# yoyololicon/spectrogram-inversion

Hardware: AMD Instinct MI355X
Metric: Griffin-Lim iterations*frames/sec at n_fft=2048 hop=512 (higher is better)
Workload: dtype f32; 1 GPU; C2: griffin_lim B64/GPU n_fft=2048 hop=512 T=1024 it=100 alpha=0.3 hann center reflect tol=0 eva_iter=10; global_batch=64, parallelism=batch-sharded x1, RCCL gather, step=phase_init + ISTFT + iterations + gather, kernel=k_fused4_td

## Files before the change

### spectrogram_inversion_amd/csrc/fast_core.h

```cpp
#pragma once
#include <algorithm>
#include <cstdlib>
#include <vector>

#include "common.h"
#include "kernels_generic.h"


namespace specinv {
namespace fast {

constexpr int kMinWaves = 2;
constexpr int kFused4Waves = 8;
constexpr int kR8Waves = 3;
constexpr double kTdsFloor = 9.3132257461547852e-10;

using v2f = float __attribute__((ext_vector_type(2)));
using v4f = float __attribute__((ext_vector_type(4)));

enum { MODE_GLA = 0, MODE_ADMM = 1 };

__device__ __forceinline__ v2f cmul_k(v2f a, v2f b) { return v2f{a.x * b.x - a.y * b.y, a.x * b.y + a.y * b.x}; }
__device__ __forceinline__ v2f cmulc_k(v2f a, v2f b) { return v2f{a.x * b.x + a.y * b.y, a.y * b.x - a.x * b.y}; }
__device__ __forceinline__ v2f cmul(v2f a, v2f b) {
// ... 531 lines not shown
  if (G::C == 4 && PK) {
#pragma unroll
    for (int g = 0; g < R; g += 4) {
      z[g] = tr[k.tr_q + (0 * R + g) * (R + 1)];
      z[g + 2] = tr[k.tr_q + (1 * R + g) * (R + 1)];
      z[g + 1] = tr[k.tr_q + (2 * R + g) * (R + 1)];
      z[g + 3] = tr[k.tr_q + (3 * R + g) * (R + 1)];
    }
#pragma unroll
    for (int g = 0; g < R; g += 4) {
      z[g + 2] = cmulc_p<PK>(z[g + 2], k.postq[0]);
      z[g + 1] = cmulc_p<PK>(z[g + 1], k.postq[1]);
      z[g + 3] = cmulc_p<PK>(z[g + 3], k.postq[2]);
    }
#pragma unroll
    for (int g = 0; g < R; g += 4) xlane_dft4_out<true>(z[g], z[g + 1], z[g + 2], z[g + 3]);
    cmul_all<R, PK, true, 1>(z, tw);
    Dft<R, true, PKC>::run(z);
    return;
  }
#pragma unroll
  for (int i = 0; i < R; ++i) z[i] = tr[k.tr_a + i * (R + 1)];
  cmul_all<R, PK, true, 0>(z, SameW{k.post});
  if (G::C == 2) {
#pragma unroll
    for (int g = 0; g < R; g += 2) xlane_dft2(z[g], z[g + 1]);
  } else if (G::C == 4) {
#pragma unroll
    for (int g = 0; g < R; g += 4) xlane_dft4<true>(z[g], z[g + 1], z[g + 2], z[g + 3]);
  } else if (G::C == 16) {
    const float s3 = (k.lane & 8) ? -1.0f : 1.0f, s2 = (k.lane & 4) ? -1.0f : 1.0f;
#pragma unroll
    for (int i = 0; i < R; ++i) {
      z[i] = cmulc_p<PK>(xlane_bf2(z[i], 4, s2), k.stage[1]);
      z[i] = cmulc_p<PK>(xlane_bf2(z[i], 8, s3), k.stage[0]);
    }
#pragma unroll
    for (int g = 0; g < R; g += 4) xlane_dft4<true>(z[g], z[g + 1], z[g + 2], z[g + 3]);
  } else {
    const bool upper = k.v & 1;
    const float sg = upper ? -1.0f : 1.0f;
#pragma unroll
    for (int i = 0; i < R; ++i) {
      const v2f p = shfl_xor2(z[i], R);
      z[i] = v2f{fmaf(z[i].x, sg, p.x), fmaf(z[i].y, sg, p.y)};
      z[i] = cmulc_p<PK>(z[i], k.stage[0]);
    }
#pragma unroll
    for (int g = 0; g < R; g += 4) xlane_dft4<true>(z[g], z[g + 1], z[g + 2], z[g + 3]);
  }
  cmul_all<R, PK, true, 1>(z, tw);
  Dft<R, true, PKC>::run(z);
}

__device__ __forceinline__ v2f w64(int j) {
  constexpr float tab[16][2] = {{1.000000000e+00f, -0.000000000e+00f}, {9.951847267e-01f, -9.801714033e-02f}, {9.807852804e-01f, -1.950903220e-01f}, {9.569403357e-01f, -2.902846773e-01f}, {9.238795325e-01f, -3.826834324e-01f}, {8.819212643e-01f, -4.713967368e-01f}, {8.314696123e-01f, -5.555702330e-01f}, {7.730104534e-01f, -6.343932842e-01f}, {7.071067812e-01f, -7.071067812e-01f}, {6.343932842e-01f, -7.730104534e-01f}, {5.555702330e-01f, -8.314696123e-01f}, {4.713967368e-01f, -8.819212643e-01f}, {3.826834324e-01f, -9.238795325e-01f}, {2.902846773e-01f, -9.569403357e-01f}, {1.950903220e-01f, -9.807852804e-01f}, {9.801714033e-02f, -9.951847267e-01f}};
  return v2f{tab[j][0], tab[j][1]};
}

struct FastArgs {
  const float* x_in;
  float* x_out;
  const float* xtail_in;
  float* xtail_out;
  const v4f* P_in;
  v4f* P_out;
  const v2f* Pmid_in;
  v2f* Pmid_out;
  v4f* X_out;
  v4f* U_out;
  v2f* Xmid_out;
  v2f* Umid_out;
  const v4f* m_pairs;
  const float* m_mid;
  const float* window;
  const float* env;
  double* partials;
  int T, nchunks, n_waves, pad_mode;
  long long L;
  const float* x2_in;
  float* x2_out;
  float tds;
  int skew;
  float coef;
  float inv1p;
  float fwd_scale;
  float inv_scale;
  v4f* P2_out;
  v2f* Pmid2_out;
  const v4f* m2_pairs;
  const float* m2_mid;
};

__device__ __forceinline__ float fast_abs(v2f s) { return __builtin_amdgcn_sqrtf(fmaf(s.x, s.x, s.y * s.y)); }
__device__ __forceinline__ float fast_rcp(float v) { return __builtin_amdgcn_rcpf(v); }
constexpr float kRefFloor = 1e-32f;
__device__ __forceinline__ float ref_norm2(v2f s, float floor_ = kRefFloor) { return fmaf(s.y, s.y, fmaf(s.x, s.x, floor_)); }
__device__ __forceinline__ v2f ref_rcp_abs2(v2f t, float guard = 1e-16f) {
  const v2f y = v2f{__builtin_amdgcn_rsqf(t.x), __builtin_amdgcn_rsqf(t.y)};
  v2f h = t * y;
  const v2f e = __builtin_elementwise_fma(-h, y, v2f{1.0f, 1.0f});
  return __builtin_elementwise_fma(y * 0.5f, e, y);
}
__device__ __forceinline__ float ref_rcp_abs(float t, float guard = 1e-16f) {
  const float y = __builtin_amdgcn_rsqf(t);
  float h = t * y;
  return fmaf(y * 0.5f, fmaf(-h, y, 1.0f), y);
}
__device__ __forceinline__ float env_rcp(float e) {
  const float r = __builtin_amdgcn_rcpf(e);
  return fmaf(fmaf(-e, r, 1.0f), r, r);
}
__device__ __forceinline__ v2f env_rcp(v2f e) { return v2f{env_rcp(e.x), env_rcp(e.y)}; }
__device__ __forceinline__ v2f env_apply_r(v2f v, v2f e, v2f r) {
  const v2f q = v * r;
  return __builtin_elementwise_fma(__builtin_elementwise_fma(-q, e, v), r, q);
}
__device__ __forceinline__ v2f env_apply(v2f v, v2f e) { return v2f{__fdiv_rn(v.x, e.x), __fdiv_rn(v.y, e.y)}; }
__device__ __forceinline__ float env_apply(float v, float e) { return __fdiv_rn(v, e); }

template <int MODE, bool EVAL>
__device__ __forceinline__ v2f update_bin(v2f r, v2f& p, v2f& u, v2f& xs, float m, const FastArgs& a, bool live, double& sd,
                                          double& so) {
  if (EVAL) {
    const float o = fast_abs(r);
    if (live) {
      const double d = (double)o - (double)m;
      sd += d * d;
      so += (double)o * (double)o;
    }
  }
  if (MODE == MODE_GLA) {
    const v2f s = v2f{fmaf(-a.coef, p.x, r.x), fmaf(-a.coef, p.y, r.y)};
    p = s;
    return ((s * m) * ref_rcp_abs(ref_norm2(s))) * a.inv_scale;
  } else {
    const v2f y = p;
    const v2f z = v2f{fmaf(a.coef, y.x, r.x) * a.inv1p, fmaf(a.coef, y.y, r.y) * a.inv1p};
    const v2f un = y - z;
    v2f xn = z - un;
    {
#pragma clang fp contract(off)
      xn = (xn * m) * ref_rcp_abs(ref_norm2(xn));
    }
    xs = xn;
    u = un;
    p = xn + un;
    return p * a.inv_scale;
  }
}

__device__ __forceinline__ long long pad_index(long long n, long long L, int pad_mode) {
  if (n >= 0 && n < L) return n;
  switch (pad_mode) {
    case SPECINV_PAD_REFLECT:
      return n < 0 ? -n : 2 * (L - 1) - n;
    case SPECINV_PAD_REPLICATE:
      return n < 0 ? 0 : L - 1;
    case SPECINV_PAD_CIRCULAR:
      return n < 0 ? n + L : n - L;
    default:
      return -1;
  }
}

__device__ __host__ __forceinline__ int chunk_begin(int c, int T, int nchunks, int skew = 0) {
// ... 228 lines not shown
```

### spectrogram_inversion_amd/csrc/fast_state.h

```cpp
#pragma once
#include <algorithm>
#include "dev_buf.h"
#include "fast_core.h"
#include "kernels_layout.h"

namespace specinv {

template <typename T>
struct FastState {
  bool supported = false;
  bool semi = false;
  bool hopk = false;
  bool xform_ok = false;
  bool two = false;
  bool keep_state = false;
  bool plain_state = false;
  int n_partials = 0;
  int nchunks = 0, skew = 0, OV = 0;
  int max_partials() const { return 0; }
  T* state_rows() const { return nullptr; }
  const T* state_tails() const { return nullptr; }
  int setup(const specinv_stft_cfg&, const std::vector<T>&, int64_t, int) { return SPECINV_OK; }
  void geometry(int out[4]) const { out[0] = out[1] = out[2] = out[3] = 0; }
  template <typename P>
  int launch_xform(P&, bool, const T*, long long, void*, T*, T, int = -1) { return fail(SPECINV_EUNSUPPORTED, "no fused path"); }
  template <typename P>
  int launch_inverse_ola(P&, const void*, T*, long long, T, T**, bool* used) {
    *used = false;
    return SPECINV_OK;
  }
  template <typename P>
  int begin(P&, int, const void*, const void*, double*) { return fail(SPECINV_EUNSUPPORTED, "no fused path for this dtype"); }
  template <typename P>
  int iterate(P&, int, bool) { return fail(SPECINV_EUNSUPPORTED, "no fused path for this dtype"); }
  template <typename P>
  int get_wave(P&, T*) { return fail(SPECINV_EUNSUPPORTED, "no fused path for this dtype"); }
  template <typename P>
  int get_state_spec(P&, int, cplx<T>*) { return fail(SPECINV_EUNSUPPORTED, "no fused path for this dtype"); }
};

#define SPECINV_R_SWITCH(RV, ...)                      \
  switch (RV) {                                        \
    case 4: { constexpr int RR = 4; __VA_ARGS__; } break;   \
    case 8: { constexpr int RR = 8; __VA_ARGS__; } break;   \
    case 16: { constexpr int RR = 16; __VA_ARGS__; } break; \
    default: { constexpr int RR = 32; __VA_ARGS__; } break; \
  }

#define SPECINV_EARLY_EVAL(early, ev, K, ...)                                                                     \
  ((early) ? ((ev) ? (const void*)K<__VA_ARGS__, true, true> : (const void*)K<__VA_ARGS__, true, false>)          \
           : ((ev) ? (const void*)K<__VA_ARGS__, false, true> : (const void*)K<__VA_ARGS__, false, false>))

struct FastKnobs {
  bool disable_fast = false;
  bool disable_twosided = false;
  bool disable_fused = false;
  bool disable_hop = false;
  bool fused_template = false;
  bool eval_kernel = true;
  bool debug = false;
  bool has_small_frames = false;
  long long small_frames = 0;
  int fast_chunk = 0;
  int cu_budget = 0;
  bool has_k4_skew = false;
  int k4_s1 = 0, k4_s2 = 0;
  bool has_td_skew = false;
  int td_skew = 0;

  static FastKnobs read() {
    auto starts = [](const char* name, char c) {
      const char* e = getenv(name);
      return e != nullptr && e[0] == c;
    };
    FastKnobs k;
    k.disable_fast = starts("SPECINV_DISABLE_FAST", '1');
    k.disable_twosided = starts("SPECINV_DISABLE_TWOSIDED", '1');
    k.disable_fused = starts("SPECINV_DISABLE_FUSED", '1');
    k.disable_hop = starts("SPECINV_DISABLE_HOP", '1');
    k.fused_template = starts("SPECINV_FUSED_TEMPLATE", '1');
    k.eval_kernel = !starts("SPECINV_EVAL_KERNEL", '0');
    k.debug = getenv("SPECINV_DEBUG") != nullptr;
    if (const char* e = getenv("SPECINV_SMALL_FRAMES")) {
      k.has_small_frames = true;
      k.small_frames = atoll(e);
    }
    if (const char* e = getenv("SPECINV_FAST_CHUNK")) k.fast_chunk = atoi(e);
    if (const char* e = getenv("SPECINV_CU_BUDGET")) k.cu_budget = atoi(e);
    if (const char* e = getenv("SPECINV_K4_SKEW")) k.has_k4_skew = sscanf(e, "%d,%d", &k.k4_s1, &k.k4_s2) == 2;
    if (const char* e = getenv("SPECINV_TD_SKEW")) {
      k.has_td_skew = true;
      k.td_skew = atoi(e);
    }
    return k;
  }
  long long frames_from(long long measured) const { return has_small_frames ? small_frames : measured; }
};

inline double chunk_cost(int batch, int n_frames, int nch, long long slots) {
  const long long waves = (long long)batch * nch;
  const long long rounds = (waves + slots - 1) / slots;
  const int longest = (n_frames + nch - 1) / nch;
  return (double)rounds * (longest + 2.0) * (1.0 + 0.0015 * std::max(0, longest - 32));
}
struct ChunkPick {
  int nch = 0;
  double cost = 1e300;
};
inline ChunkPick pick_chunks(int batch, int n_frames, long long slots, int lo, int hi, int mult = 1, double tie = 1e-9) {
  ChunkPick best;
  for (int nch = lo; nch <= hi; ++nch) {
    if (nch % mult != 0) continue;
    const double cost = chunk_cost(batch, n_frames, nch, slots);
    if (cost < best.cost + tie) best = ChunkPick{nch, cost};
  }
  return best;
}

enum FastKernel {
  kKernelFused4 = 1,
  kKernelFused = 2,
  kKernelSemi = 3,
  kKernelHop = 4,
  kKernelFused4Td = 5,
  kKernelFusedTd = 6,
  kKernelHopTd = 7,
};

template <>
struct FastState<float> {
  using v2f = fast::v2f;
  using v4f = fast::v4f;
  bool supported = false;
  bool semi = false;
  bool hopk = false;
  int semi_grid = 0;
  int R = 0;
  int OV = 0;
  FastKnobs knobs;
  int chunk = 32, nchunks = 0, n_waves = 0, n_partials = 0;
  int skew = 0;
  int cur = 0;
  int mode = fast::MODE_GLA;
  DevBuf xb[2], xtail[2], Pb, Pmid, mpairs, mmid, scratch;
  bool two = false;
  DevBuf Pb2, Pmid2, mpairs2, mmid2;
  bool keep_state = false, xu_valid = false;
  DevBuf Xb, Xmid, Ub, Umid;
  bool plain_state = false;
  float* state_rows() const { return xb[cur].template as<float>(); }
  const float* state_tails() const { return (!semi && nchunks > 1) ? xtail[cur].template as<float>() : nullptr; }
  bool td = false;
  int td_t = 0;
  DevBuf zb[2];

  template <typename P>
  int want_xu(P& pl, fast::FastArgs& a, bool last) {
    if (mode != fast::MODE_ADMM) return SPECINV_OK;
    xu_valid = false;
    if (!keep_state || !last) return SPECINV_OK;
    SI_TRY(reserve_xu(pl));
    a.X_out = Xb.template as<v4f>();
    a.U_out = Ub.template as<v4f>();
    a.Xmid_out = Xmid.template as<v2f>();
// ... 19 lines not shown
    if (cfg.dtype != SPECINV_F32) return SPECINV_OK;
    knobs = FastKnobs::read();
    if (knobs.disable_fast) return SPECINV_OK;
    const bool size_ok = cfg.n_fft == 512 || cfg.n_fft == 1024 || cfg.n_fft == 2048 || cfg.n_fft == 4096;
    if (!size_ok) return SPECINV_OK;
    if (!cfg.onesided) {
      if (knobs.disable_twosided) return SPECINV_OK;
      if (pad >= length) return SPECINV_OK;
      two = true;
    } else {
      xform_ok = true;
      xform_R = cfg.n_fft / 128;
    }
    R = cfg.n_fft / 128;
    semi = false;
    OV = 0;
    for (int o : {2, 4, 8})
      if (cfg.hop_length * o == cfg.n_fft && R % o == 0) OV = o;
    if (two || knobs.disable_fused) OV = 0;
    const long long n_all = (long long)cfg.batch * cfg.n_frames;
    const bool small = n_all < knobs.frames_from(6144);
    if (!cfg.center || OV == 0 || cfg.n_frames < OV + 2 || pad >= length || small) {
      semi = true;
      hopk = false;
      OV = 0;
      chunk = cfg.n_frames;
      nchunks = 1;
      semi_grid = (int)std::min<long long>((n_all + 3) / 4, 256 * 8);
      n_waves = semi_grid * 4;
      supported = true;
      const bool want_hop = !knobs.disable_hop && R <= 16 && n_all >= knobs.frames_from(R >= 16 ? 12288 : 32768) && !small &&
                            cfg.hop_length >= 1 && cfg.hop_length <= cfg.n_fft && pad < length;
      if (want_hop) {
        const int floor_ch = std::max(8, (cfg.n_fft - 1) / cfg.hop_length + 1);
        const long long slots = R >= 16 ? 2048 : R == 8 ? 4096 : 6144;
        hopk = true;
        nchunks = pick_chunks(cfg.batch, cfg.n_frames, slots, 1, std::max(1, cfg.n_frames / floor_ch)).nch;
        if (knobs.fast_chunk >= 1) nchunks = std::max(1, cfg.n_frames / std::min(std::max(knobs.fast_chunk, floor_ch), cfg.n_frames));
        chunk = (cfg.n_frames + nchunks - 1) / nchunks;
        n_waves = cfg.batch * nchunks;
        if (knobs.debug) fprintf(stderr, "specinv: frame kernel with LDS overlap-add R=%d hop=%d chunks=%d of <=%d frames, %d waves\n", R, cfg.hop_length, nchunks, chunk, n_waves);
      }
      return SPECINV_OK;
    }
    const int floor_ch = OV == 8 ? 16 : 8;
    long long slots = 1024LL * (R >= 32 ? 1 : R <= 4 ? 3 : 2);
    if (R == 8) slots = 1024LL * fast::kR8Waves;
    if (knobs.cu_budget > 0 && knobs.cu_budget < 256) slots = slots * (256 - knobs.cu_budget) / 256;
    const int most = std::max(1, cfg.n_frames / floor_ch);
    ChunkPick best = pick_chunks(cfg.batch, cfg.n_frames, slots, 1, most);
    if (OV == 4 && (R == 16 || R == 8)) {
      const int mult = R == 16 ? 2 : 3;
      if (best.nch % mult != 0) {
        const ChunkPick pick = pick_chunks(cfg.batch, cfg.n_frames, slots, std::max(mult, best.nch - mult), std::min(best.nch + mult, most), mult, 0.0);
        if (pick.nch > 0 && pick.cost <= 1.04 * best.cost) best = pick;
      }
    }
    nchunks = best.nch;
    if (knobs.fast_chunk >= 4) nchunks = std::max(1, cfg.n_frames / std::min(std::max(knobs.fast_chunk, OV == 8 ? 13 : 4), cfg.n_frames));
    chunk = (cfg.n_frames + nchunks - 1) / nchunks;
    n_waves = cfg.batch * nchunks;
    if (knobs.debug) fprintf(stderr, "specinv: fused R=%d OV=%d chunks=%d of <=%d frames, %d waves (%lld slots)\n", R, OV, nchunks, chunk, n_waves, slots);
    supported = true;
    return SPECINV_OK;
  }

  template <typename P>
  fast::FastArgs base_args(P& pl) const {
    fast::FastArgs a{};
    a.m_pairs = mpairs.template as<v4f>();
    a.m_mid = mmid.template as<float>();
    if (two) {
      a.P2_out = Pb2.template as<v4f>();
      a.Pmid2_out = Pmid2.template as<v2f>();
      a.m2_pairs = mpairs2.template as<v4f>();
      a.m2_mid = mmid2.template as<float>();
    }
    a.window = pl.window.template as<float>();
    a.env = pl.env.template as<float>();
    a.partials = pl.partials_out();
    a.T = pl.Tn();
    a.nchunks = nchunks;
    a.skew = skew;
    a.n_waves = n_waves;
    a.pad_mode = pl.cfg.pad_mode;
    a.L = pl.length;
    a.coef = pl.coef;
    a.inv1p = 1.0f / (float)(1.0 + (double)pl.coef);
    a.fwd_scale = pl.fc.fwd_scale;
    a.inv_scale = pl.fc.inv_scale;
    return a;
  }

  template <typename P, typename A>
  static int launch_waves(P& pl, const void* fn, const A& args, int waves, int wgw, size_t lds) {
    SI_HIP(hipFuncSetAttribute(fn, hipFuncAttributeMaxDynamicSharedMemorySize, (int)lds));
    A copy = args;
    void* kargs[] = {&copy};
    SI_HIP(hipLaunchKernel(fn, dim3((waves + wgw - 1) / wgw), dim3(64 * wgw), kargs, lds, pl.stream));
    return SPECINV_OK;
  }

  template <int RR, typename P>
  int begin_t(P& pl, int md, const v2f* spec_user, const float* mag_user, double* sum_m2_out) {
    using G = fast::Geo<RR>;
    const int hop = pl.cfg.hop_length;
    mode = md;
    td = md == fast::MODE_GLA && (!semi || hopk) && !knobs.fused_template && !keep_state && !plain_state && RR <= 16 && !two;
    if (pl.cfg.normalized && !hopk) td = false;
    const bool emit_pairs = ((hop | pl.pad) & 1) == 0 && (pl.length & 1) == 0;
    int hop_td_max = emit_pairs ? (RR == 4 ? 320 : RR == 8 ? 1024 : 800) : (RR == 4 ? 128 : RR == 8 ? 448 : 416);
    if (hopk && hop > hop_td_max) td = false;
    td_t = 0;
    skew = 0;
    {
      const int len_ch = pl.Tn() / std::max(1, nchunks);
      if (td && !semi && RR == 16 && OV == 4 && n_waves > 1024 && (nchunks & 1) == 0 && len_ch >= 12) {
        constexpr int kSkewC2 = 10;
        skew = n_waves == 2048 && len_ch == 32 ? kSkewC2 : std::min((len_ch + 2) / 4, len_ch - 8);
        if (skew < 2) skew = 0;
      }
      if (!semi && RR == 8 && OV == 4 && !knobs.fused_template && fused_wgw() == 12 && nchunks % 3 == 0 && len_ch >= 16) {
        constexpr int kSkew1 = 4, kSkew2 = 6;
        const int s1 = len_ch == 64 ? kSkew1 : (kSkew1 * len_ch + 32) / 64;
        const int s2 = len_ch == 64 ? kSkew2 : (kSkew2 * len_ch + 32) / 64;
        if ((s1 | s2) && len_ch - s2 >= 8 && len_ch + s2 - s1 >= 8) skew = 0x10000 | (s1 << 8) | s2;
      }
    }
    if (knobs.has_k4_skew) {
      const int s1 = knobs.k4_s1, s2 = knobs.k4_s2;
      if (!semi && fused_wgw() == 12 && nchunks % 3 == 0 && n_waves % 12 == 0 && s1 >= 0 && s2 >= 0 && s1 < 200 && s2 < 200 &&
          pl.Tn() / nchunks - s2 >= 8 && pl.Tn() / nchunks + s2 - s1 >= 8)
        skew = (s1 | s2) ? (0x10000 | (s1 << 8) | s2) : 0;
    }
    if (knobs.has_td_skew) {
      const int v = knobs.td_skew;
      if (v == 0 || (td && !semi && (nchunks & 1) == 0 && (n_waves & 1) == 0 && pl.Tn() / nchunks - v >= 8)) skew = v;
    }
    if (td) {
      SI_TRY(zb[0].reserve((size_t)pl.B() * pl.length * sizeof(float)));
      SI_TRY(zb[1].reserve((size_t)pl.B() * pl.length * sizeof(float)));
    }
    const long long nf = (long long)pl.B() * pl.Tn();
    const size_t pbytes = (size_t)nf * G::H * 64 * sizeof(v4f);
    const size_t tail_bytes = (size_t)pl.B() * nchunks * (OV > 0 ? OV - 1 : 0) * hop * sizeof(float);
    if (hopk) SI_TRY(xtail[0].reserve((size_t)pl.B() * nchunks * (pl.N() - hop) * sizeof(float) + 16));
    for (int i = 0; i < ((semi && !hopk) ? 1 : 2); ++i) {
      if (!semi) SI_TRY(xtail[i].reserve(tail_bytes));
      SI_TRY(xb[i].reserve((size_t)pl.B() * pl.length * sizeof(float)));
    }
    SI_TRY(Pb.reserve(pbytes));
    SI_TRY(Pmid.reserve(nf * sizeof(v2f)));
    if (semi && !hopk) SI_TRY(pl.frames_needed());
    SI_TRY(mpairs.reserve((size_t)nf * (G::H / 2) * 64 * sizeof(v4f)));
    SI_TRY(mmid.reserve(nf * sizeof(float)));
    if (two) {
      SI_TRY(Pb2.reserve(pbytes));
      SI_TRY(Pmid2.reserve(nf * sizeof(v2f)));
      SI_TRY(mpairs2.reserve((size_t)nf * (G::H / 2) * 64 * sizeof(v4f)));
      SI_TRY(mmid2.reserve(nf * sizeof(float)));
    }
    cur = 0;
    SI_CHECK(!two || spec_user != nullptr, SPECINV_ESTATE, "the two-sided frame kernel takes its starting spectrum in the user layout");
    if (spec_user == nullptr) {
      const int nwg = pl.B() * G::H;
      SI_TRY(pl.partials.reserve(std::max<size_t>((size_t)nwg, 3 * 1024) * sizeof(double)));
// ... 428 lines not shown
```

### spectrogram_inversion_amd/csrc/kernels_fast_td.h

```cpp
#pragma once
#include "fast_core.h"

namespace specinv {
namespace fast {


template <bool FIRST, typename A, typename B>
__device__ __forceinline__ const auto& td_pick(const A& a, const B& b) {
  if constexpr (FIRST) return a;
  else return b;
}


template <int R, int OV, bool NT = false>
__device__ __forceinline__ void td_load_block(const float* __restrict__ xrow, const float* __restrict__ tailrow, long long L,
                                              int T, int c, int t_begin, int t_end, int j, int lane, int pad_mode,
                                              v2f (&q)[R / OV]) {
  if constexpr (OV == 4) load_block4<R, NT>(xrow, tailrow, L, T, c, t_begin, t_end, j, lane, pad_mode, q);
  else load_block<R, OV>(xrow, tailrow, L, T, c, t_begin, t_end, j, lane, pad_mode, q);
}

using lds_v2f = __attribute__((address_space(3))) v2f;
struct TdScratch {
  volatile lds_v2f* q;
  lds_v2f* b;
};
template <int R>
__device__ __forceinline__ TdScratch td_scratch(v2f* tr, const LaneConst<R>& k) {
  TdScratch s;
  s.q = (volatile lds_v2f*)(tr + k.tr_q);
  s.b = (lds_v2f*)(tr + k.tr_b);
  asm volatile("" : "+v"(s.b));
  return s;
}

template <bool INV>
__device__ __forceinline__ void dft4_rot2(v2f& a0, v2f& a1, v2f& a2, v2f& a3) {
  const v2f t0 = INV ? add_i(a0, a2) : sub_i(a0, a2);
  const v2f t1 = INV ? sub_i(a0, a2) : add_i(a0, a2);
  const v2f t2 = a1 + a3, d = a1 - a3;
  a0 = t0 + t2;
  a2 = t0 - t2;
  a1 = INV ? add_i(t1, d) : sub_i(t1, d);
  a3 = INV ? sub_i(t1, d) : add_i(t1, d);
}
template <bool INV>
__device__ __forceinline__ void td_dft16(v2f (&a)[16]) {
  constexpr float c1 = 0.92387953251128675613f, s1 = 0.38268343236508977173f, h = 0.70710678118654752440f;
#pragma unroll
  for (int n0 = 0; n0 < 4; ++n0) dft4<INV>(a[n0], a[n0 + 4], a[n0 + 8], a[n0 + 12]);
  dirmul_x4<INV, true>(a[5], a[6], a[7], a[9], v2f{c1, -s1}, v2f{h, -h}, v2f{s1, -c1}, v2f{h, -h});
  dirmul_x4<INV, true>(a[11], a[13], a[14], a[15], v2f{-h, -h}, v2f{s1, -c1}, v2f{-h, -h}, v2f{-c1, s1});
  dft4<INV>(a[0], a[1], a[2], a[3]);
  dft4<INV>(a[4], a[5], a[6], a[7]);
  dft4_rot2<INV>(a[8], a[9], a[10], a[11]);
  dft4<INV>(a[12], a[13], a[14], a[15]);
  v2f o[16];
#pragma unroll
  for (int k0 = 0; k0 < 4; ++k0)
#pragma unroll
    for (int k1 = 0; k1 < 4; ++k1) o[k1 + 4 * k0] = a[k0 + 4 * k1];
#pragma unroll
  for (int i = 0; i < 16; ++i) a[i] = o[i];
}

template <int R, typename TW>
__device__ __forceinline__ void td_fft_forward(v2f (&z)[R], const LaneConst<R>& k, const TW& tw, v2f* __restrict__ tr,
                                               const TdScratch& sc) {
  if constexpr (R == 16) {
    td_dft16<false>(z);
    cmul_all<R, true, false, 1>(z, tw);
#pragma unroll
    for (int g = 0; g < R; g += 4) xlane_dft4_in<false>(z[g], z[g + 1], z[g + 2], z[g + 3]);
#pragma unroll
    for (int g = 0; g < R; g += 4) {
      z[g + 2] = cmul(z[g + 2], k.postq[0]);
      z[g + 1] = cmul(z[g + 1], k.postq[1]);
      z[g + 3] = cmul(z[g + 3], k.postq[2]);
    }
#pragma unroll
    for (int g = 0; g < R; g += 4) {
      sc.q[(0 * R + g) * (R + 1)] = z[g];
      sc.q[(1 * R + g) * (R + 1)] = z[g + 2];
      sc.q[(2 * R + g) * (R + 1)] = z[g + 1];
      sc.q[(3 * R + g) * (R + 1)] = z[g + 3];
    }
#pragma unroll
    for (int i = 0; i < R; ++i) z[i] = sc.b[i];
    td_dft16<false>(z);
  } else {
    fft_forward_t<R>(z, k, tw, tr);
  }
}
template <int R, typename TW>
__device__ __forceinline__ void td_fft_inverse(v2f (&z)[R], const LaneConst<R>& k, const TW& tw, v2f* __restrict__ tr,
                                               const TdScratch& sc) {
  if constexpr (R == 16) {
    td_dft16<true>(z);
#pragma unroll
    for (int i = 0; i < R; ++i) sc.b[i] = z[i];
#pragma unroll
    for (int g = 0; g < R; g += 4) {
// ... 46 lines not shown
  v2f* lds_tw1 = lds_win + 2 * M;
  const int wib = __builtin_amdgcn_readfirstlane(threadIdx.x >> 6);
  v2f* tr = lds_tw1 + (R - 1) * 64 + wib * G::TR;

  WinRegs<M> wreg;
  win_request<M>(a.window, wreg);
  for (int i = threadIdx.x; i < (R - 1) * 64; i += blockDim.x) {
    const int k1 = i / 64 + 1, l = i & 63;
    lds_tw1[i] = unit(2.0f * (float)((l * k1) % M) / (float)M);
  }
  win_store<M>(wreg, lds_win, lds_wins, a.inv_scale);
  __syncthreads();

  int w = __builtin_amdgcn_readfirstlane(blockIdx.x * (blockDim.x >> 6) + wib);
  if (a.skew == 0 && w >= a.n_waves) return;
  const LaneConst<R> k = lane_consts<R>();
  const TdScratch tsc = td_scratch<R>(tr, k);
  const int lane = k.lane;
  const unsigned ulane = (unsigned)lane;
  int b = w / a.nchunks, c = w - b * a.nchunks;
  if (a.skew >= 0x10000) {
    const int cg = 3 * ((int)blockIdx.x * 4 + (wib & 3)) + (wib >> 2);
    b = cg / a.nchunks;
    c = cg - b * a.nchunks;
    w = cg;
  } else if (a.skew != 0 && (blockDim.x >> 6) == 8) {
    const int cg = 2 * ((int)blockIdx.x * 4 + (wib & 3)) + (wib >> 2);
    b = cg / a.nchunks;
    c = cg - b * a.nchunks;
    w = cg;
  } else if (a.skew != 0) {
    const int half = a.n_waves >> 1, second = w >= half ? 1 : 0, wl = w - second * half, pairs = a.nchunks >> 1;
    b = wl / pairs;
    c = 2 * (wl - b * pairs) + second;
    w = b * a.nchunks + c;
  }
  if (a.skew != 0 && w >= a.n_waves) return;
  const int t_begin = chunk_begin(c, a.T, a.nchunks, a.skew);
  const int t_end = chunk_begin(c + 1, a.T, a.nchunks, a.skew);
  const float* zrow = a.x_in + (long long)b * a.L;
  const float* tailrow = a.xtail_in + (long long)b * a.nchunks * NB * HOP;
  float* zorow = a.x_out + (long long)b * a.L;
  const bool write_x = a.x2_out != nullptr;
  float* xorow = a.x2_out + (long long)b * a.L;
  const float half_scale = 0.5f * a.fwd_scale;
  const float tds_raw = a.tds / half_scale;
  const float nlr = -a.coef;

  v2f acc[NB * QU];
#pragma unroll
  for (int i = 0; i < NB * QU; ++i) acc[i] = v2f{0.0f, 0.0f};
  double sd = 0.0, so = 0.0;
  constexpr bool TWLDS = EVAL && R >= 16;
  TwRegs<TWLDS ? 2 : R> twr_regs;
  if (!TWLDS) {
#pragma unroll
    for (int k1 = 1; k1 < R; ++k1) twr_regs.w[(TWLDS ? 1 : k1) - 1] = lds_tw1[(k1 - 1) * 64 + lane];
  }
  const TwLds twr_lds{lds_tw1, lane};
  const auto& twr = td_pick<TWLDS>(twr_lds, twr_regs);

  v2f xq[NB][QU], xn[QU];
#pragma unroll
  for (int q = 0; q < NB; ++q)
    td_load_block<R, OV, true>(zrow, tailrow, a.L, a.T, c, t_begin, t_end, t_begin + q, lane, a.pad_mode, xq[q]);
  td_load_block<R, OV, true>(zrow, tailrow, a.L, a.T, c, t_begin, t_end, t_begin + NB, lane, a.pad_mode, xn);

  constexpr bool ENVREG = !EVAL;
  v2f envc[QU], envr[QU];
  if (ENVREG) {
    const v2f* e0 = reinterpret_cast<const v2f*>(a.env + (long long)(NB - PB) * HOP);
#pragma unroll
    for (int i = 0; i < QU; ++i) {
      envc[i] = e0[64u * i + ulane];
      envr[i] = env_rcp(envc[i]);
    }
  }
  constexpr bool WKREG = !EVAL;
  v2f wkr[WKREG ? H : 1];
  if (WKREG) {
#pragma unroll
    for (int j = 0; j < H; ++j) wkr[j] = pair_twiddle<R>(k.wn, j);
  }
  for (int t = t_begin; t < t_end; ++t) {
    asm volatile("" ::: "memory");
    v2f wn = k.wn;
    if (!WKREG) asm volatile("" : "+v"(wn));
    const long long fi = (long long)b * a.T + t;
    v4f mm[H / 2];
    v4f pp[EARLY ? H : 1];
    v2f pmid = v2f{0.0f, 0.0f};
    float mmid = 0.0f;
    __builtin_amdgcn_s_setprio(1);
    {
      const v4f* min_ = a.m_pairs + fi * (H / 2 * 64);
#pragma unroll
      for (int j = 0; j < H / 2; ++j) mm[j] = ld_stream(&min_[j * 64u + ulane]);
      if (lane == 0) {
        mmid = a.m_mid[fi];
        if (EARLY) pmid = a.Pmid_in[fi];
      }
    }
#define SPECINV_TD_C0_LOADS()                                                              \
    if (EARLY) {                                                                           \
      const v4f* pin_ = a.P_in + fi * (H * 64);                                            \
      _Pragma("unroll") for (int j = 0; j < H; ++j) pp[j] = ld_stream(&pin_[j * 64u + ulane]); \
    }
    if (!EVAL) SPECINV_TD_C0_LOADS();

    v2f z[R];
    if (EVAL) {
      const float* xrow = a.x2_in + (long long)b * a.L;
#pragma unroll
      for (int qq = 0; qq < OV; ++qq) {
        v2f q[QU];
        td_load_block<R, OV>(xrow, tailrow, a.L, a.T, c, t_begin, t_end, t + qq, lane, a.pad_mode, q);
#pragma unroll
        for (int i = 0; i < QU; ++i) z[qq * QU + i] = q[i] * lds_win[64 * (qq * QU + i) + lane];
      }
      td_fft_forward<R>(z, k, twr, tr, tsc);
      v2f rc[H];
#pragma unroll
      for (int m = H; m < R; ++m) {
        const v2f got = shfl2(z[m], k.partner);
        const v2f own = z[(m + 1) % R];
        rc[m - H] = v2f{lane == 0 ? own.x : got.x, lane == 0 ? own.y : got.y};
      }
      float fd = 0.0f, fo = 0.0f;
#pragma unroll
      for (int j = 0; j < H; ++j) {
        const v2f wk = pair_twiddle<R>(wn, j);
        v2f xk, xm;
        td_split<R>(z[j], rc[R - 1 - j - H], wk, half_scale, xk, xm);
        const float mk = (j & 1) ? mm[j / 2].z : mm[j / 2].x;
        const float mq = (j & 1) ? mm[j / 2].w : mm[j / 2].y;
        const float ok = fast_abs(xk), om = fast_abs(xm);
        const float dk = ok - mk, dm = om - mq;
        fd = fmaf(dk, dk, fmaf(dm, dm, fd));
        fo = fmaf(ok, ok, fmaf(om, om, fo));
      }
      if (lane == 0) {
        const float o = fast_abs(z[H] * v2f{a.fwd_scale, -a.fwd_scale});
        const float d = o - mmid;
        fd = fmaf(d, d, fd);
        fo = fmaf(o, o, fo);
      }
      sd += (double)fd;
      so += (double)fo;
      asm volatile("" ::: "memory");
      __builtin_amdgcn_sched_barrier(0);
      SPECINV_TD_C0_LOADS();
    }
#undef SPECINV_TD_C0_LOADS

    v2f zold[QU];
#pragma unroll
    for (int i = 0; i < QU; ++i) {
      zold[i] = xq[0][i];
#pragma unroll
      for (int q = 0; q < NB; ++q) z[q * QU + i] = xq[q][i] * lds_win[64 * (q * QU + i) + lane];
      z[NB * QU + i] = xn[i] * lds_win[64 * (NB * QU + i) + lane];
#pragma unroll
      for (int q = 0; q + 1 < NB; ++q) xq[q][i] = xq[q + 1][i];
      xq[NB - 1][i] = xn[i];
    }
    if (t + 1 < t_end) {
      td_load_block<R, OV, true>(zrow, tailrow, a.L, a.T, c, t_begin, t_end, t + OV, lane, a.pad_mode, xn);
    } else {
#pragma unroll
      for (int i = 0; i < QU; ++i) asm volatile("" : "=v"(xn[i]));
    }
    __builtin_amdgcn_s_setprio(0);

    td_fft_forward<R>(z, k, twr, tr, tsc);

    v2f rc[H];
    if constexpr (R == 16) {
#pragma unroll
      for (int m = H; m < R; ++m) rc[m - H] = shfl2(z[m], k.partner);
      td_lane0_mov8(rc[0], rc[1], rc[2], rc[3], rc[4], rc[5], rc[6], rc[7], z[9], z[10], z[11], z[12], z[13], z[14], z[15], z[0]);
    } else {
#pragma unroll
      for (int m = H; m < R; ++m) {
        const v2f got = shfl2(z[m], k.partner);
        const v2f own = z[(m + 1) % R];
        rc[m - H] = v2f{lane == 0 ? own.x : got.x, lane == 0 ? own.y : got.y};
      }
    }

    v2f back[H];
    {
      v2f sk[H], sm[H], tt[H], yy[H], hh[H];
#pragma unroll
      for (int j = 0; j < H; ++j) {
        const v2f wk = WKREG ? wkr[WKREG ? j : 0] : pair_twiddle<R>(wn, j);
        td_split_raw<R>(z[j], rc[R - 1 - j - H], wk, sk[j], sm[j]);
        if (EARLY) {
          sk[j] = __builtin_elementwise_fma(v2f{pp[j].x, pp[j].y}, v2f{tds_raw, tds_raw}, sk[j]);
          sm[j] = __builtin_elementwise_fma(v2f{pp[j].z, pp[j].w}, v2f{tds_raw, tds_raw}, sm[j]);
        }
        tt[j] = v2f{ref_norm2(sk[j], 4.0f * kRefFloor), ref_norm2(sm[j], 4.0f * kRefFloor)};
      }
#pragma unroll
      for (int j = 0; j < H; ++j) yy[j] = v2f{__builtin_amdgcn_rsqf(tt[j].x), __builtin_amdgcn_rsqf(tt[j].y)};
#pragma unroll
      for (int j = 0; j < H; ++j) hh[j] = tt[j] * yy[j];
#pragma unroll
      for (int j = 0; j < H; ++j) tt[j] = __builtin_elementwise_fma(-hh[j], yy[j], v2f{1.0f, 1.0f});
#pragma unroll
      for (int j = 0; j < H; ++j) yy[j] = __builtin_elementwise_fma(yy[j] * 0.5f, tt[j], yy[j]);
#pragma unroll
      for (int j = 0; j < H; ++j) {
        const v2f mp = (j & 1) ? v2f{mm[j / 2].z, mm[j / 2].w} : v2f{mm[j / 2].x, mm[j / 2].y};
        sk[j] = scale_lo(sk[j], mp);
        sm[j] = scale_hi(sm[j], mp);
      }
#pragma unroll
      for (int j = 0; j < H; ++j) {
        const v2f wk = WKREG ? wkr[WKREG ? j : 0] : pair_twiddle<R>(wn, j);
        v2f ak = scale_lo(sk[j], yy[j]);
        v2f am = scale_hi(sm[j], yy[j]);
        if (j == 0 && lane == 0) {
          ak.y = 0.0f;
          am.y = 0.0f;
        }
        const v2f e2i = add_conj(ak, am);
        const v2f o2i = cmulc(sub_conj(ak, am), wk);
        z[j] = add_i(e2i, o2i);
        back[j] = conj_sub_i(e2i, o2i);
      }
    }
    v2f zmid;
    {
      v2f smid = z[H] * v2f{a.fwd_scale, -a.fwd_scale};
      if (EARLY) smid = v2f{fmaf(a.tds, pmid.x, smid.x), fmaf(a.tds, pmid.y, smid.y)};
      const v2f am = (smid * mmid) * ref_rcp_abs(ref_norm2(smid));
      zmid = am * v2f{2.0f, -2.0f};
    }
    if constexpr (R == 16) {
#pragma unroll
      for (int m = H; m < R; ++m) z[m] = shfl2(back[R - 1 - m], k.partner);
      td_lane0_mov8(z[8], z[9], z[10], z[11], z[12], z[13], z[14], z[15], zmid, back[7], back[6], back[5], back[4], back[3], back[2],
                    back[1]);
    } else {
#pragma unroll
      for (int m = H; m < R; ++m) {
        const v2f got = shfl2(back[R - 1 - m], k.partner);
        const v2f l0 = (m == H) ? zmid : back[(R - m) % H];
        z[m] = v2f{lane == 0 ? l0.x : got.x, lane == 0 ? l0.y : got.y};
      }
    }

    td_fft_inverse<R>(z, k, twr, tr, tsc);

#pragma unroll
    for (int u = 0; u < NB * QU; ++u) z[u] = z[u] * lds_wins[64 * u + lane];
    if (t >= PB) {
      const long long o0 = (long long)(t - PB) * HOP;
      const v2f* envp = reinterpret_cast<const v2f*>(a.env + o0);
      v2f* xo = reinterpret_cast<v2f*>(xorow + o0);
      v2f* zo = reinterpret_cast<v2f*>(zorow + o0);
      if (!ENVREG) {
#pragma unroll
        for (int i = 0; i < QU; ++i) {
          envc[i] = envp[64u * i + ulane];
          envr[i] = env_rcp(envc[i]);
        }
      } else if (t <= NB) {
#pragma unroll
        for (int i = 0; i < QU; ++i) envc[i] = envp[64u * i + ulane];
#pragma unroll
        for (int i = 0; i < QU; ++i) asm volatile("" : "+v"(envc[i]));
#pragma unroll
        for (int i = 0; i < QU; ++i) envr[i] = env_rcp(envc[i]);
      }
#pragma unroll
      for (int i = 0; i < QU; ++i) {
        const v2f xv = env_apply_r(acc[i] + z[i], envc[i], envr[i]);
        const v2f zv = __builtin_elementwise_fma(v2f{nlr, nlr}, zold[i], xv);
        if (write_x) xo[64u * i + ulane] = xv;
        zo[64u * i + ulane] = zv;
      }
    }
#pragma unroll
    for (int i = 0; i < QU; ++i) {
#pragma unroll
      for (int q = 0; q + 1 < NB; ++q) acc[q * QU + i] = acc[(q + 1) * QU + i] + z[(q + 1) * QU + i];
    }
#pragma unroll
    for (int i = 0; i < QU; ++i) acc[(NB - 1) * QU + i] = z[NB * QU + i] * lds_wins[64 * (NB * QU + i) + lane];
  }
  if (t_end == a.T) {
#pragma unroll
    for (int q = 0; q < PB - 1; ++q) {
      const long long o0 = (long long)(a.T + q - PB) * HOP;
      const v2f* envp = reinterpret_cast<const v2f*>(a.env + o0);
      v2f* xo = reinterpret_cast<v2f*>(xorow + o0);
      v2f* zo = reinterpret_cast<v2f*>(zorow + o0);
#pragma unroll
      for (int i = 0; i < QU; ++i) {
        const v2f xv = env_apply(acc[q * QU + i], envp[64u * i + ulane]);
        if (write_x) xo[64u * i + ulane] = xv;
        zo[64u * i + ulane] = v2f{fmaf(nlr, xq[q][i].x, xv.x), fmaf(nlr, xq[q][i].y, xv.y)};
      }
    }
  } else {
    v2f* tl = reinterpret_cast<v2f*>(a.xtail_out + ((long long)b * a.nchunks + c) * NB * HOP);
#pragma unroll
    for (int q = 0; q < NB; ++q) {
      const v2f* envp = reinterpret_cast<const v2f*>(a.env + (long long)(t_end + q - PB) * HOP);
#pragma unroll
      for (int i = 0; i < QU; ++i) tl[(q * QU + i) * 64u + ulane] = env_apply(acc[q * QU + i], envp[64u * i + ulane]);
    }
  }
  if (EVAL) {
    const double d = wave_sum(sd), o = wave_sum(so);
    if (lane == 0) {
      a.partials[2 * (long long)w] = d;
      a.partials[2 * (long long)w + 1] = o;
    }
  }
}

template <int R, bool EARLY, bool EVAL>
__global__ __launch_bounds__(R == 8 ? 768 : 64 * kFused4Waves, R == 8 ? kR8Waves : kMinWaves) void k_fused4_td(FastArgs a) {
  fused_td_body<R, 4, EARLY, EVAL>(a);
}
template <int R, int OV, bool EARLY, bool EVAL>
__global__ __launch_bounds__(256, R >= 32 ? 1 : R == 8 ? kR8Waves : kMinWaves) void k_fused_td(FastArgs a) {
  fused_td_body<R, OV, EARLY, EVAL>(a);
}

constexpr int kEvalSub = kEvalPieces;
template <int R, int OV>
__global__ __launch_bounds__(256, kEvalWaves) void k_eval_td(FastArgs a) {
  using G = Geo<R>;
  using O = Ovl<R, OV>;
  constexpr int H = G::H, M = G::M, QU = O::QU, HOP = O::HOP, NB = O::NB;
  extern __shared__ __attribute__((aligned(16))) char smem[];
  v2f* lds_win = reinterpret_cast<v2f*>(smem);
  v2f* lds_tw1 = lds_win + M;
  const int wib = __builtin_amdgcn_readfirstlane(threadIdx.x >> 6);
  v2f* tr = lds_tw1 + (R - 1) * 64 + wib * G::TR;
  WinRegs<M> wreg;
  win_request<M>(a.window, wreg);
  for (int i = threadIdx.x; i < (R - 1) * 64; i += blockDim.x) {
    const int k1 = i / 64 + 1, l = i & 63;
    lds_tw1[i] = unit(2.0f * (float)((l * k1) % M) / (float)M);
  }
  win_store<M>(wreg, lds_win);
  __syncthreads();
  const int w = __builtin_amdgcn_readfirstlane(blockIdx.x * 4 + wib);
  if (w >= a.n_waves * kEvalSub) return;
  const LaneConst<R> k = lane_consts<R>();
  const TdScratch tsc = td_scratch<R>(tr, k);
  const int lane = k.lane;
  const unsigned ulane = (unsigned)lane;
  const int cw = w / kEvalSub, sub = w - cw * kEvalSub;
  const int b = cw / a.nchunks, c = cw - b * a.nchunks;
  const int t_begin = chunk_begin(c, a.T, a.nchunks, a.skew), t_end = chunk_begin(c + 1, a.T, a.nchunks, a.skew);
  const int s_begin = t_begin + (sub * (t_end - t_begin)) / kEvalSub, s_end = t_begin + ((sub + 1) * (t_end - t_begin)) / kEvalSub;
  const float* xrow = a.x2_in + (long long)b * a.L;
  const float* tailrow = a.xtail_in + (long long)b * a.nchunks * NB * HOP;
  const float half_scale = 0.5f * a.fwd_scale;
  TwRegs<R> twr;
#pragma unroll
  for (int k1 = 1; k1 < R; ++k1) twr.w[k1 - 1] = lds_tw1[(k1 - 1) * 64 + lane];
  double sd = 0.0, so = 0.0;
  v2f xq[NB][QU], xn[QU];
#pragma unroll
  for (int q = 0; q < NB; ++q)
    td_load_block<R, OV>(xrow, tailrow, a.L, a.T, c, t_begin, t_end, s_begin + q, lane, a.pad_mode, xq[q]);
  td_load_block<R, OV>(xrow, tailrow, a.L, a.T, c, t_begin, t_end, s_begin + NB, lane, a.pad_mode, xn);
// ... 69 lines not shown
```

Baseline: 336.7 million iterations*frames/s.

## Peel steady-state frames in TD kernel with boundary-free loads and target prefetch

Splits the per-frame loop of the fused time-domain Griffin-Lim kernel into a generic path and a steady-state interior path, via a lambda templated on a steady tag. Interior frames load overlapping signal blocks without padding or boundary checks and skip the edge-only envelope branches. They also issue the next frame's target-magnitude loads early, in the middle of the current frame's spectral work, to hide memory latency. The cost is larger code, more live registers because the prefetched magnitudes stay resident, and a new env knob (on by default) that applies only to non-eval launches with OV=4 and R of 8 or 16.

```diff
diff --git a/spectrogram_inversion_amd/csrc/fast_core.h b/spectrogram_inversion_amd/csrc/fast_core.h
--- a/spectrogram_inversion_amd/csrc/fast_core.h
+++ b/spectrogram_inversion_amd/csrc/fast_core.h
@@ -637,6 +637,7 @@
   float* x2_out;
   float tds;
   int skew;
+  int td_steady;
   float coef;
   float inv1p;
   float fwd_scale;
diff --git a/spectrogram_inversion_amd/csrc/fast_state.h b/spectrogram_inversion_amd/csrc/fast_state.h
--- a/spectrogram_inversion_amd/csrc/fast_state.h
+++ b/spectrogram_inversion_amd/csrc/fast_state.h
@@ -67,6 +67,7 @@
   int k4_s1 = 0, k4_s2 = 0;
   bool has_td_skew = false;
   int td_skew = 0;
+  bool td_steady = true;
 
   static FastKnobs read() {
     auto starts = [](const char* name, char c) {
@@ -80,6 +81,7 @@
     k.disable_hop = starts("SPECINV_DISABLE_HOP", '1');
     k.fused_template = starts("SPECINV_FUSED_TEMPLATE", '1');
     k.eval_kernel = !starts("SPECINV_EVAL_KERNEL", '0');
+    k.td_steady = !starts("SPECINV_TD_STEADY", '0');
     k.debug = getenv("SPECINV_DEBUG") != nullptr;
     if (const char* e = getenv("SPECINV_SMALL_FRAMES")) {
       k.has_small_frames = true;
@@ -265,6 +267,7 @@
     a.T = pl.Tn();
     a.nchunks = nchunks;
     a.skew = skew;
+    a.td_steady = knobs.td_steady ? 1 : 0;
     a.n_waves = n_waves;
     a.pad_mode = pl.cfg.pad_mode;
     a.L = pl.length;
diff --git a/spectrogram_inversion_amd/csrc/kernels_fast_td.h b/spectrogram_inversion_amd/csrc/kernels_fast_td.h
--- a/spectrogram_inversion_amd/csrc/kernels_fast_td.h
+++ b/spectrogram_inversion_amd/csrc/kernels_fast_td.h
@@ -1,4 +1,6 @@
 #pragma once
+#include <type_traits>
+
 #include "fast_core.h"
 
 namespace specinv {
@@ -18,6 +20,21 @@
                                               v2f (&q)[R / OV]) {
   if constexpr (OV == 4) load_block4<R, NT>(xrow, tailrow, L, T, c, t_begin, t_end, j, lane, pad_mode, q);
   else load_block<R, OV>(xrow, tailrow, L, T, c, t_begin, t_end, j, lane, pad_mode, q);
+}
+
+template <int R, int OV>
+__device__ __forceinline__ void td_load_interior(const float* __restrict__ xrow, int j, unsigned ulane, v2f (&q)[R / OV]) {
+  using O = Ovl<R, OV>;
+  const v2f* src = reinterpret_cast<const v2f*>(xrow + (long long)(j - O::PB) * O::HOP);
+#pragma unroll
+  for (int i = 0; i < O::QU; ++i) q[i] = __builtin_nontemporal_load(&src[64u * i + ulane]);
+}
+template <int R>
+__device__ __forceinline__ void td_request_target(const v4f* __restrict__ m_pairs, long long fi, unsigned ulane,
+                                                  v4f (&mm)[Geo<R>::H / 2]) {
+  const v4f* min_ = m_pairs + fi * (Geo<R>::H / 2 * 64);
+#pragma unroll
+  for (int j = 0; j < Geo<R>::H / 2; ++j) mm[j] = ld_stream(&min_[j * 64u + ulane]);
 }
 
 using lds_v2f = __attribute__((address_space(3))) v2f;
@@ -230,20 +247,20 @@
 #pragma unroll
     for (int j = 0; j < H; ++j) wkr[j] = pair_twiddle<R>(k.wn, j);
   }
-  for (int t = t_begin; t < t_end; ++t) {
+  v4f mm[H / 2];
+  auto frame = [&](auto steady_tag, const int t) __attribute__((always_inline)) {
+    constexpr bool STEADY = decltype(steady_tag)::value;
+    constexpr bool AHEAD = STEADY;
     asm volatile("" ::: "memory");
     v2f wn = k.wn;
     if (!WKREG) asm volatile("" : "+v"(wn));
     const long long fi = (long long)b * a.T + t;
-    v4f mm[H / 2];
     v4f pp[EARLY ? H : 1];
     v2f pmid = v2f{0.0f, 0.0f};
     float mmid = 0.0f;
     __builtin_amdgcn_s_setprio(1);
     {
-      const v4f* min_ = a.m_pairs + fi * (H / 2 * 64);
-#pragma unroll
-      for (int j = 0; j < H / 2; ++j) mm[j] = ld_stream(&min_[j * 64u + ulane]);
+      if (!AHEAD) td_request_target<R>(a.m_pairs, fi, ulane, mm);
       if (lane == 0) {
         mmid = a.m_mid[fi];
         if (EARLY) pmid = a.Pmid_in[fi];
@@ -312,7 +329,9 @@
       for (int q = 0; q + 1 < NB; ++q) xq[q][i] = xq[q + 1][i];
       xq[NB - 1][i] = xn[i];
     }
-    if (t + 1 < t_end) {
+    if (STEADY) {
+      td_load_interior<R, OV>(zrow, t + OV, ulane, xn);
+    } else if (t + 1 < t_end) {
       td_load_block<R, OV, true>(zrow, tailrow, a.L, a.T, c, t_begin, t_end, t + OV, lane, a.pad_mode, xn);
     } else {
 #pragma unroll
@@ -363,6 +382,7 @@
         sk[j] = scale_lo(sk[j], mp);
         sm[j] = scale_hi(sm[j], mp);
       }
+      if (AHEAD) td_request_target<R>(a.m_pairs, fi + 1, ulane, mm);
 #pragma unroll
       for (int j = 0; j < H; ++j) {
         const v2f wk = WKREG ? wkr[WKREG ? j : 0] : pair_twiddle<R>(wn, j);
@@ -403,7 +423,7 @@
 
 #pragma unroll
     for (int u = 0; u < NB * QU; ++u) z[u] = z[u] * lds_wins[64 * u + lane];
-    if (t >= PB) {
+    if (STEADY || t >= PB) {
       const long long o0 = (long long)(t - PB) * HOP;
       const v2f* envp = reinterpret_cast<const v2f*>(a.env + o0);
       v2f* xo = reinterpret_cast<v2f*>(xorow + o0);
@@ -414,7 +434,7 @@
           envc[i] = envp[64u * i + ulane];
           envr[i] = env_rcp(envc[i]);
         }
-      } else if (t <= NB) {
+      } else if (!STEADY && t <= NB) {
 #pragma unroll
         for (int i = 0; i < QU; ++i) envc[i] = envp[64u * i + ulane];
 #pragma unroll
@@ -437,6 +457,18 @@
     }
 #pragma unroll
     for (int i = 0; i < QU; ++i) acc[(NB - 1) * QU + i] = z[NB * QU + i] * lds_wins[64 * (NB * QU + i) + lane];
+  };
+  constexpr bool HAS_STEADY = !EVAL && OV == 4 && (R == 8 || R == 16);
+  const int st_end = t_end - OV;
+  const int st_begin = (HAS_STEADY && a.td_steady != 0 && std::max(t_begin, NB + 1) < st_end) ? std::max(t_begin, NB + 1) : t_end;
+  for (int t = t_begin; t < t_end; ++t) {
+    if constexpr (HAS_STEADY) {
+      if (t == st_begin) {
+        td_request_target<R>(a.m_pairs, (long long)b * a.T + t, ulane, mm);
+        for (; t < st_end; ++t) frame(std::true_type{}, t);
+      }
+    }
+    frame(std::false_type{}, t);
   }
   if (t_end == a.T) {
 #pragma unroll
```

New measurement: 337.5 million iterations*frames/s (median of 3 runs). About the same (+0.2%).
